# zhai-lw/L3AC

Hardware: AMD Instinct MI355X
Metric: audio samples/sec encode+decode, 1kbps@16kHz, batch 256; indices bit-exact (higher is better)
Workload: dtype f32

## Files before the change

include/l3ac_hip.h:

```cpp
#ifndef L3AC_HIP_H
#define L3AC_HIP_H

#include <stddef.h>
#include <stdint.h>

#ifdef __cplusplus
extern "C" {
#endif

#define L3AC_ABI_VERSION 5
#define L3AC_MAX_STAGES 8
#define L3AC_MAX_LEVELS 8

enum {
    L3AC_OK = 0,
    L3AC_EINVAL = -1,
    L3AC_EWEIGHT = -2,
    L3AC_EHIP = -3,
    L3AC_ENOMEM = -4,
    L3AC_ECOOP = -5,
};

typedef struct l3ac_config {
    int32_t abi_version;
// ... 94 lines not shown
int l3ac_op_enhance_up(l3ac_ctx* ctx, const char* enhance_block, const char* up_block, const float* x, int32_t batch,
                       int32_t frames, float* y, void* stream);
int l3ac_op_last_block(l3ac_ctx* ctx, const float* x, int32_t batch, int32_t frames, float* audio, void* stream);
int l3ac_op_legacy_unit(l3ac_ctx* ctx, int32_t unit, const float* x, int32_t batch, int32_t frames, float* y, void* stream);
int l3ac_op_head(l3ac_ctx* ctx, const float* x, int32_t batch, int32_t frames, float* audio, void* stream);
int l3ac_op_local_trans(l3ac_ctx* ctx, const char* block, const float* x, int32_t batch, int32_t frames, float* y,
                        void* stream);
int l3ac_op_encoder(l3ac_ctx* ctx, const float* audio, int32_t batch, int32_t samples, float* feature, void* stream);
int l3ac_op_en_encoder(l3ac_ctx* ctx, const float* feature, int32_t batch, int32_t frames, float* tokens, void* stream);
int l3ac_op_en_decoder(l3ac_ctx* ctx, const float* tokens, int32_t batch, int32_t n_tok, float* feature, void* stream);
int l3ac_op_decoder(l3ac_ctx* ctx, const float* feature, int32_t batch, int32_t frames, float* audio, void* stream);

int l3ac_op_snake(const float* x, float* y, int64_t rows, int32_t c, const float* alpha, int32_t mode, void* stream);
int l3ac_ctx_set_head_pretanh(l3ac_ctx* ctx, int32_t enable);

typedef struct l3ac_profile_entry {
    char name[64];
    int32_t launches;
    int32_t reserved;
    double ms_total;
    double flops;
    double bytes;
} l3ac_profile_entry;
int l3ac_profile_begin(void);
int l3ac_profile_end(l3ac_profile_entry* out, int32_t cap, int32_t* n_out);

int l3ac_gemm_f32(const float* a, int64_t lda, const float* w, const float* bias, float* c, int64_t ldc,
                  int64_t m, int32_t n, int32_t k, void* stream);

void l3ac_split3_host(const float* x, int64_t n, uint16_t* planes);
int l3ac_ctx_set_gemm_split(l3ac_ctx* ctx, int32_t enable);
int l3ac_ctx_set_option(l3ac_ctx* ctx, const char* name, int32_t value);
int l3ac_ctx_get_option(const l3ac_ctx* ctx, const char* name, int32_t* out);
int32_t l3ac_ctx_get_gemm_split(const l3ac_ctx* ctx);
int64_t l3ac_gemm_split_image_bytes(int32_t n, int32_t k);
int l3ac_gemm_split_image(const float* w, int32_t n, int32_t k, void* image, void* stream);
int l3ac_gemm_split_f32(const float* a, int64_t lda, const void* image, const float* bias, float* c, int64_t ldc,
                        int64_t m, int32_t n, int32_t k, void* stream);
int l3ac_gemm_split_f32_at(const float* a, int64_t lda, const void* image, const float* bias, float* c, int64_t ldc,
                           int64_t m, int32_t n, int32_t k, int32_t w256, void* stream);

#ifdef __cplusplus
}
#endif
#endif
```

l3ac_amd/_capi.py:

```python
from __future__ import annotations

import ctypes as C
from pathlib import Path

import os

LIB_PATH = Path(os.environ.get("L3AC_LIB_PATH") or Path(__file__).resolve().parent / "libl3ac_hip.so")
ABI_VERSION = 5
MAX_STAGES = 8
MAX_LEVELS = 8


class L3acError(RuntimeError):
    pass


class Config(C.Structure):
    _fields_ = [
        ("abi_version", C.c_int32),
        ("feature_dim", C.c_int32),
        ("n_enc", C.c_int32),
        ("enc_dims", C.c_int32 * MAX_STAGES),
        ("enc_depths", C.c_int32 * MAX_STAGES),
        ("compress_rates", C.c_int32 * MAX_STAGES),
# ... 31 lines not shown
    "l3ac_encode": (C.c_int, [_P, _P, _I32, _I32, _I64, _P, _P, _P, _P]),
    "l3ac_decode": (C.c_int, [_P, _P, _P, _I32, _I32, _P, _P]),
    "l3ac_encode_ragged": (C.c_int, [_P, _P, _I32, _I32, _I64, C.POINTER(_I32), _P, _P, _P, _P]),
    "l3ac_decode_ragged": (C.c_int, [_P, _P, _P, _I32, _I32, C.POINTER(_I32), _P, _P]),
    "l3ac_fsq_forward": (C.c_int, [_P, _I64, _I32, C.POINTER(_I32), _I32, _P, _P, _P, _P, _P, _P, _P, _P, _P]),
    "l3ac_fsq_quantize_act": (C.c_int, [_P, _I64, _I32, C.POINTER(_I32), _I32, _P, _P, _P, _P, _P, _P]),
    "l3ac_fsq_decode": (C.c_int, [_P, _I64, _I32, C.POINTER(_I32), _I32, _P, _P, _P, _P]),
    "l3ac_fsq_copy_ceiling": (C.c_int, [_P, _I64, _P, _P, _P, _P]),
    "l3ac_fsq_copy_ceiling_at": (C.c_int, [_P, _I64, _P, _P, _P, _I32, _P]),
    "l3ac_vq_argmin_scratch_bytes": (_I64, [_I64, _I32, _I32]),
    "l3ac_vq_argmin": (C.c_int, [_P, _I64, _P, _I32, _I32, _P, _P, _I64, _I32, _P]),
    "l3ac_op_first_block": (C.c_int, [_P, _P, _I32, _I32, _P, _P]),
    "l3ac_op_conv_unit": (C.c_int, [_P, C.c_char_p, _P, _I32, _I32, _P, _P]),
    "l3ac_op_down_layer": (C.c_int, [_P, C.c_char_p, _P, _I32, _I32, _P, _P]),
    "l3ac_op_conv_k3": (C.c_int, [_P, C.c_char_p, _P, _I32, _I32, _P, _P]),
    "l3ac_op_enhance": (C.c_int, [_P, C.c_char_p, _P, _I32, _I32, _P, _P]),
    "l3ac_op_up_layer": (C.c_int, [_P, C.c_char_p, _P, _I32, _I32, _P, _P]),
    "l3ac_op_enhance_up": (C.c_int, [_P, C.c_char_p, C.c_char_p, _P, _I32, _I32, _P, _P]),
    "l3ac_op_last_block": (C.c_int, [_P, _P, _I32, _I32, _P, _P]),
    "l3ac_op_legacy_unit": (C.c_int, [_P, _I32, _P, _I32, _I32, _P, _P]),
    "l3ac_op_head": (C.c_int, [_P, _P, _I32, _I32, _P, _P]),
    "l3ac_op_local_trans": (C.c_int, [_P, C.c_char_p, _P, _I32, _I32, _P, _P]),
    "l3ac_op_encoder": (C.c_int, [_P, _P, _I32, _I32, _P, _P]),
    "l3ac_op_en_encoder": (C.c_int, [_P, _P, _I32, _I32, _P, _P]),
    "l3ac_op_en_decoder": (C.c_int, [_P, _P, _I32, _I32, _P, _P]),
    "l3ac_op_decoder": (C.c_int, [_P, _P, _I32, _I32, _P, _P]),
    "l3ac_op_snake": (C.c_int, [_P, _P, _I64, _I32, _P, _I32, _P]),
    "l3ac_ctx_set_head_pretanh": (C.c_int, [_P, _I32]),
    "l3ac_gemm_f32": (C.c_int, [_P, _I64, _P, _P, _P, _I64, _I64, _I32, _I32, _P]),
    "l3ac_split3_host": (None, [_P, _I64, _P]),
    "l3ac_ctx_set_gemm_split": (C.c_int, [_P, _I32]),
    "l3ac_ctx_set_option": (C.c_int, [_P, C.c_char_p, _I32]),
    "l3ac_ctx_get_option": (C.c_int, [_P, C.c_char_p, C.POINTER(_I32)]),
    "l3ac_ctx_get_gemm_split": (_I32, [_P]),
    "l3ac_gemm_split_image_bytes": (_I64, [_I32, _I32]),
    "l3ac_gemm_split_image": (C.c_int, [_P, _I32, _I32, _P, _P]),
    "l3ac_gemm_split_f32": (C.c_int, [_P, _I64, _P, _P, _P, _I64, _I64, _I32, _I32, _P]),
    "l3ac_gemm_split_f32_at": (C.c_int, [_P, _I64, _P, _P, _P, _I64, _I64, _I32, _I32, _I32, _P]),
    "l3ac_pack_indices": (C.c_int, [_P, _I32, _I32, _I32, _P, _I32, _P]),
    "l3ac_unpack_indices": (C.c_int, [_P, _I32, _I32, _I32, _I32, _P, _P]),
    "l3ac_resample_length": (_I64, [_I32, _I32, _I64]),
    "l3ac_resample_bank": (_I64, [_I32, _I32, _P, _I64]),
    "l3ac_resample": (C.c_int, [_P, _I32, _I64, _I64, _I32, _I32, _P, _P, _I64, _P]),
    "l3ac_profile_begin": (C.c_int, []),
    "l3ac_profile_end": (C.c_int, [_P, _I32, C.POINTER(_I32)]),
}


class ProfileEntry(C.Structure):
    _fields_ = [("name", C.c_char * 64), ("launches", C.c_int32), ("reserved", C.c_int32),
                ("ms_total", C.c_double), ("flops", C.c_double), ("bytes", C.c_double)]


class profile:

    def __enter__(self):
        check(load_library().l3ac_profile_begin())
        self.entries = []
        return self

    def __exit__(self, *exc):
        buf = (ProfileEntry * 64)()
        n = C.c_int32(0)
        check(load_library().l3ac_profile_end(buf, 64, C.byref(n)))
        self.entries = [dict(name=buf[i].name.decode(), launches=buf[i].launches, ms_total=buf[i].ms_total,
                             flops=buf[i].flops, bytes=buf[i].bytes) for i in range(n.value)]
# ... 104 lines not shown
        return int(out.value)

    def coop_timeout_pending(self) -> int:
        out = _I64(0)
        check(self.lib.l3ac_coop_timeout_pending(self.handle, C.byref(out)))
        return int(out.value)

    def grn_min_norm(self, reset: bool = False) -> float:
        out = C.c_float(0.0)
        check(self.lib.l3ac_grn_min_norm(self.handle, int(reset), C.byref(out)))
        return float(out.value)

    @property
    def workspace_bytes(self) -> int:
        return self.lib.l3ac_workspace_bytes(self.handle)

    def reserve(self, batch: int, samples: int) -> None:
        check(self.lib.l3ac_reserve(self.handle, batch, samples))

    def set_gemm_split(self, enable: bool) -> None:
        check(self.lib.l3ac_ctx_set_gemm_split(self.handle, int(bool(enable))))

    def get_gemm_split(self) -> bool:
        return bool(self.lib.l3ac_ctx_get_gemm_split(self.handle))

    def set_option(self, name: str, value: int) -> None:
        check(self.lib.l3ac_ctx_set_option(self.handle, name.encode(), int(value)))

    def get_option(self, name: str) -> int:
        out = _I32(0)
        check(self.lib.l3ac_ctx_get_option(self.handle, name.encode(), C.byref(out)))
        return int(out.value)

    def set_head_pretanh(self, enable: bool) -> None:
        check(self.lib.l3ac_ctx_set_head_pretanh(self.handle, int(bool(enable))))
```

l3ac_amd/csrc/capi.hip:

```cpp
#include <algorithm>
#include <cmath>
#include <cstdarg>
#include <cstdlib>
#include <cstring>
#include <new>
#include <string>
#include <vector>

#include "network.hpp"
#include "kernels/split_bf16.hpp"

static thread_local std::string g_last_error;

void l3ac_set_error(const char* fmt, ...) {
    char buf[1024];
    va_list ap;
    va_start(ap, fmt);
    vsnprintf(buf, sizeof(buf), fmt, ap);
    va_end(ap);
    g_last_error = buf;
}

int l3ac_device_cu_count() {
    static std::atomic<int> cus[L3AC_MAX_DEVICES] = {};
// ... 97 lines not shown
template <class Map>
auto lookup(const Map& m, const char* name, const char* kind) -> decltype(m.begin()->second) {
    if (!name) {
        l3ac_set_error("null block name");
        return nullptr;
    }
    auto it = m.find(name);
    if (it == m.end()) {
        l3ac_set_error("no %s block named '%s'", kind, name);
        return nullptr;
    }
    return it->second;
}

struct Option {
    const char* name;
    int& (*field)(l3ac_ctx&);
    bool flag;
    int lo, hi, def;
    const char* env;
};
#define L3AC_FIELD(member) [](l3ac_ctx& c) -> int& { return c.member; }
const Option kOptions[] = {
    {"gemm_split", L3AC_FIELD(gemm_split), true, 0, 1, 1, "L3AC_GEMM_SPLIT"},
    {"head_pretanh", L3AC_FIELD(head_pretanh), true, 0, 1, 0, nullptr},
    {"narrow_ring", L3AC_FIELD(narrow_ring), false, 0, 2, 1, nullptr},
    {"wide_sliced", L3AC_FIELD(wide_sliced), false, 0, 2, 1, nullptr},
    {"unit_counter", L3AC_FIELD(unit_counter), false, 0, 3, 1, "L3AC_UNIT_COUNTER"},
    {"trans_coop", L3AC_FIELD(coop.enabled), true, 0, 1, 1, "L3AC_TRANS_COOP"},
    {"coop_timeout_ms", L3AC_FIELD(coop.timeout_ms), false, 1, 20000, 250, nullptr},
    {"down_fused", L3AC_FIELD(down_fused), false, 0, 2, 2, "L3AC_DOWN_FUSED"},
    {"gemm_w256", L3AC_FIELD(gemm_w256), false, 0, 2, 1, "L3AC_GEMM_W256"},
    {"unit_chunk_mb", L3AC_FIELD(unit_chunk_mb), false, 0, 65536, 192, "L3AC_UNIT_CHUNK_MB"},
};
#undef L3AC_FIELD

const Option* find_option(const char* name) {
    for (const Option& o : kOptions)
        if (std::strcmp(o.name, name) == 0) return &o;
    return nullptr;
}

int unknown_option(const char* who, const char* name) {
    std::string names;
    for (const Option& o : kOptions) names += std::string(names.empty() ? "" : ", ") + o.name;
    l3ac_set_error("%s: unknown option '%s' (%s; to set only: coop_release_claim, coop_test_fault)", who, name, names.c_str());
    return L3AC_EINVAL;
}

int initial_value(const Option& o) {
    const char* e = o.env ? std::getenv(o.env) : nullptr;
    return e ? std::atoi(e) : o.def;
}

int checked_value(const Option& o, int value) { return o.flag ? value != 0 : std::min(std::max(value, o.lo), o.hi); }

int set_checked(l3ac_ctx* ctx, const Option& o, int value, const char* who) {
    L3AC_REQUIRE(!(std::strcmp(o.name, "down_fused") == 0 && value == 1),
                 "%s: down_fused = 1 (the bf16x3 one-kernel down layers) was retired, DESIGN.md section 4; 2 (the default) is the one-kernel "
                 "form with the bits of 0, the GEMM + row kernel", who);
    o.field(*ctx) = checked_value(o, value);
    return L3AC_OK;
}

int ragged_plan(l3ac_ctx* ctx, hipStream_t s, RaggedPlan& p, int batch, int max_tok, const int32_t* n_tok, const int32_t* samples) {
    p.max_tok = max_tok;
// ... 576 lines not shown
    int rc = L3AC_OK;
    if (hipMemcpyAsync(inv, hi.data(), (size_t)c * sizeof(float), hipMemcpyHostToDevice, s) != hipSuccess) {
        l3ac_set_error("op_snake: upload failed");
        rc = L3AC_EHIP;
    }
    if (rc == L3AC_OK) rc = launch_snake(s, x, y, rows, c, alpha, inv, mode);
    (void)hipStreamSynchronize(s);
    (void)hipFree(inv);
    return rc;
}

int l3ac_ctx_set_option(l3ac_ctx* ctx, const char* name, int32_t value) {
    L3AC_REQUIRE(ctx != nullptr && name != nullptr, "set_option: null argument");
    if (std::strcmp(name, "coop_release_claim") == 0) {
        trans_coop_release(ctx->coop);
        return L3AC_OK;
    }
    if (std::strcmp(name, "coop_test_fault") == 0) {
        ctx->coop.fault_part = value - 1;
        return L3AC_OK;
    }
    const Option* o = find_option(name);
    return o ? set_checked(ctx, *o, value, "set_option") : unknown_option("set_option", name);
}

int l3ac_ctx_get_option(const l3ac_ctx* ctx, const char* name, int32_t* out) {
    L3AC_REQUIRE(ctx != nullptr && name != nullptr && out != nullptr, "get_option: null argument");
    const Option* o = find_option(name);
    if (!o) return unknown_option("get_option", name);
    *out = o->field(const_cast<l3ac_ctx&>(*ctx));
    return L3AC_OK;
}

int l3ac_ctx_set_gemm_split(l3ac_ctx* ctx, int32_t enable) { return l3ac_ctx_set_option(ctx, "gemm_split", enable); }
int32_t l3ac_ctx_get_gemm_split(const l3ac_ctx* ctx) { int32_t v = 0; return l3ac_ctx_get_option(ctx, "gemm_split", &v) == L3AC_OK ? v : 0; }

int64_t l3ac_gemm_split_image_bytes(int32_t n, int32_t k) {
    return (n > 0 && k > 0 && gemm_split_eligible(n, k)) ? gemm_split_image_bytes(n, k) : 0;
}

int l3ac_gemm_split_image(const float* w, int32_t n, int32_t k, void* image, void* stream) {
    L3AC_REQUIRE(gemm_split_eligible(n, k), "split image: shape n=%d k=%d is not eligible (n >= 192, k >= 32, k %% 8 == 0)", n, k);
    return launch_gemm_split_image((hipStream_t)stream, w, k, n, k, (unsigned char*)image);
}

int l3ac_gemm_split_f32_at(const float* a, int64_t lda, const void* image, const float* bias, float* c, int64_t ldc, int64_t m,
                           int32_t n, int32_t k, int32_t w256, void* stream) {
    L3AC_REQUIRE(w256 >= 0 && w256 <= 2, "split gemm: w256 = %d, not 0, 1 or 2", w256);
    GemmArgs g{};
    g.a = a; g.lda = lda; g.w_img = (const unsigned char*)image; g.c = c; g.ldc = ldc; g.m = m; g.n = n; g.k = k; g.bias = bias;
    g.epi = EPI_BIAS; g.w256 = w256;
    return launch_gemm_split((hipStream_t)stream, g);
}
int l3ac_gemm_split_f32(const float* a, int64_t lda, const void* image, const float* bias, float* c, int64_t ldc, int64_t m,
                        int32_t n, int32_t k, void* stream) {
    const Option& o = *find_option("gemm_w256");
    return l3ac_gemm_split_f32_at(a, lda, image, bias, c, ldc, m, n, k, checked_value(o, initial_value(o)), stream);
}

}
```

l3ac_amd/csrc/network.hip:

```cpp
#include "network.hpp"

#include <algorithm>
#include <cmath>
#include <cstring>

namespace {

constexpr int HEADS = 6;

struct Builder {
    std::unordered_map<std::string, const l3ac_tensor*> map;
    std::vector<float> host;
    float* dev = nullptr;
    size_t cap = 0;
    std::string err;
    struct GemmWeight { const float* d; int n, k; };
    std::vector<GemmWeight> gemm_ws;
    struct ExtraImage { std::vector<unsigned char> bytes; const unsigned char** target; };
    std::vector<ExtraImage> extra_imgs;
    const float* host_of(const float* d) const { return host.data() + (d - dev); }

    const float* gemm(const float* d, int n, int k) {
        if (d && gemm_split_eligible(n, k)) gemm_ws.push_back({d, n, k});
        return d;
    }
    const float* find(const std::string& name, int64_t numel) {
        auto it = map.find(name);
        if (it == map.end()) {
            if (err.empty()) err = "missing weight tensor '" + name + "'";
            return nullptr;
        }
        if (it->second->numel != numel) {
            if (err.empty())
// ... 696 lines not shown
    g.w = w.w; g.ldw = 3 * w.cin; g.c = y; g.ldc = w.cout; g.m = (int64_t)batch * frames; g.n = w.cout; g.k = 3 * w.cin;
    g.bias = w.b; g.epi = EPI_BIAS;
    (void)ctx;
    return gemm_on_route(ctx, s, g);
}

int run_enhance(l3ac_ctx* ctx, hipStream_t s, const EnhW& w, const float* x, float* y, int batch, int frames) {
    Workspace& ws = ctx->ws;
    const RaggedClips rc = ctx->rag ? ctx->rag->clips(frames) : RaggedClips{};
    L3AC_TRY(launch_enhance_branches(s, w.t, x, batch, frames, w.c, ws.yi, ctx->rag ? &rc : nullptr));
    L3AC_TRY(launch_enhance_stats(s, ws.yi, batch, frames, ws.stats, ctx->rag ? &rc : nullptr));
    RowArgs r{};
    r.x = x; r.y = y; r.batch = batch; r.frames_in = frames; r.frames_out = frames; r.c = w.c;
    r.src = SRC_GATE; r.norm = NORM_NONE; r.yi = ws.yi; r.stats = ws.stats; r.in_w = w.in_w; r.in_b = w.in_b;
    r.gate_w = w.gate_w; r.gate_b = w.gate_b;
    return launch_rows(s, r);
}

int run_up(l3ac_ctx* ctx, hipStream_t s, const UpW& w, const float* x, float* tmp, float* y, int batch, int frames) {
    GemmArgs g{};
    g.a = x; g.lda = w.cin; g.w = w.w; g.ldw = w.cin; g.c = tmp; g.ldc = w.cout; g.m = (int64_t)batch * frames; g.n = w.cout; g.k = w.cin;
    g.bias = w.b; g.epi = EPI_BIAS;
    L3AC_TRY(gemm_on_route(ctx, s, g));
    L3AC_TRY(rag_dup(ctx, s, tmp, batch, frames, w.cout));
    RowArgs r{};
    r.x = tmp; r.y = y; r.batch = batch; r.frames_in = frames; r.frames_out = (int64_t)frames * w.scale; r.c = w.cout;
    r.src = SRC_LERP; r.scale = w.scale; r.norm = NORM_CN; r.nw = w.nw; r.nb = w.nb; r.eps = 1e-8f;
    (void)ctx;
    return launch_rows(s, r);
}

static bool use_up_fused(const l3ac_ctx* ctx, const UpW& w) { return ctx->gemm_split && w.fused_img != nullptr; }

int run_enhance_up(l3ac_ctx* ctx, hipStream_t s, const EnhW& e, const UpW& w, float* x, float* tmp, float* y, int batch, int frames) {
    const bool wide_up = ctx->img(w.w) != nullptr && gemm_split_eligible(w.cout, w.cin);
    if (w.cin % 16 != 0 || e.c != w.cin || wide_up) {
        L3AC_REQUIRE(tmp != nullptr, "enhance_up: scratch missing");
        float* gated = x;
        if (x != y) {
            L3AC_REQUIRE((size_t)batch * frames * e.c <= ctx->ws.h_cap, "enhance_up: workspace too small for the gated rows");
            gated = ctx->ws.h;
        }
        L3AC_TRY(run_enhance(ctx, s, e, x, gated, batch, frames));
        return run_up(ctx, s, w, gated, tmp, y, batch, frames);
    }
    Workspace& ws = ctx->ws;
    const RaggedClips rc = ctx->rag ? ctx->rag->clips(frames) : RaggedClips{};
    L3AC_TRY(launch_enhance_branches(s, e.t, x, batch, frames, e.c, ws.yi, ctx->rag ? &rc : nullptr));
    L3AC_TRY(launch_enhance_stats(s, ws.yi, batch, frames, ws.stats, ctx->rag ? &rc : nullptr));
    if (use_up_fused(ctx, w) && x != y) {
        L3AC_TRY(rag_dup(ctx, s, x, batch, frames, e.c));
        L3AC_TRY(rag_dup(ctx, s, ws.yi, batch, frames, 4));
        return launch_up_fused(s, e, w, x, ws.yi, ws.stats, y, batch, frames);
    }
    L3AC_REQUIRE(tmp != nullptr, "enhance_up: scratch missing");
    GemmArgs g{};
    g.a = x; g.lda = w.cin; g.w = w.w; g.ldw = w.cin; g.c = tmp; g.ldc = w.cout; g.m = (int64_t)batch * frames; g.n = w.cout; g.k = w.cin;
    g.bias = w.b; g.epi = EPI_BIAS;
    g.gate_yi = ws.yi; g.gate_stats = ws.stats; g.gate_in_w = e.in_w; g.gate_in_b = e.in_b; g.gate_w = e.gate_w; g.gate_b = e.gate_b;
    g.gate_frames = frames;
    L3AC_TRY(launch_gemm(s, g));
    L3AC_TRY(rag_dup(ctx, s, tmp, batch, frames, w.cout));
    RowArgs r{};
    r.x = tmp; r.y = y; r.batch = batch; r.frames_in = frames; r.frames_out = (int64_t)frames * w.scale; r.c = w.cout;
    r.src = SRC_LERP; r.scale = w.scale; r.norm = NORM_CN; r.nw = w.nw; r.nb = w.nb; r.eps = 1e-8f;
    return launch_rows(s, r);
}

static bool last_block_fused(const l3ac_ctx* ctx) {
    int max_dil = 1;
    for (const LegacyW& l : ctx->legacy) max_dil = l.dil > max_dil ? l.dil : max_dil;
    return last_block_fused_supported(ctx->head.c, max_dil);
}

int run_legacy_unit(l3ac_ctx* ctx, hipStream_t s, const LegacyW& l, const float* x, float* y, int batch, int frames) {
    if (last_block_fused(ctx))
        return launch_legacy_unit_fused(s, l, x, y, batch, frames, ctx->gemm_split, ctx->unit_counter == 1 || ctx->unit_counter == 3 ? ctx->wide_counters + 4 : nullptr);
    Workspace& ws = ctx->ws;
    const int64_t rows = (int64_t)batch * frames;
    L3AC_TRY(launch_snake(s, x, ws.a, rows, l.c, l.a0, l.ia0));
    GemmArgs g{};
    g.a = ws.a; g.lda = l.c; g.taps = 7; g.dil = l.dil; g.cin = l.c; g.frames = frames;
    g.w = l.w1; g.ldw = 7 * l.c; g.c = ws.h; g.ldc = l.c; g.m = rows; g.n = l.c; g.k = 7 * l.c;
    g.bias = l.b1; g.epi = EPI_SNAKE; g.alpha = l.a1; g.inv_alpha = l.ia1;
    L3AC_TRY(gemm_on_route(ctx, s, g));
    GemmArgs g2{};
    g2.a = ws.h; g2.lda = l.c; g2.w = l.w2; g2.ldw = l.c; g2.c = y; g2.ldc = l.c; g2.m = rows; g2.n = l.c; g2.k = l.c;
    g2.bias = l.b2; g2.epi = EPI_BIAS_RES; g2.res = x; g2.ldres = l.c;
    return gemm_on_route(ctx, s, g2);
}

int run_head(l3ac_ctx* ctx, hipStream_t s, const float* x, float* audio, int batch, int frames) {
// ... 66 lines not shown
        RowArgs r{};
        r.x = x; r.y = ws.a; r.batch = batch; r.frames_in = frames; r.frames_out = frames; r.c = dim;
        r.src = SRC_PLAIN; r.norm = NORM_LN; r.nw = l.ln1w; r.nb = l.ln1b; r.eps = 1e-5f;
        L3AC_TRY(launch_rows(s, r));
        GemmArgs g{};
        g.a = ws.a; g.lda = dim; g.w = l.wqkv; g.ldw = dim; g.c = ws.h; g.ldc = 3 * ctx->inner; g.m = rows; g.n = 3 * ctx->inner; g.k = dim;
        g.epi = EPI_BIAS;
        L3AC_TRY(gemm_on_route(ctx, s, g));
        L3AC_TRY(launch_attention(s, ws.h, ws.a, w.bias_table, batch, frames, HEADS, ctx->dim_head, w.window));
        GemmArgs go{};
        go.a = ws.a; go.lda = ctx->inner; go.w = l.wout; go.ldw = ctx->inner; go.c = x; go.ldc = dim; go.m = rows; go.n = dim; go.k = ctx->inner;
        go.epi = EPI_BIAS_RES; go.res = x; go.ldres = dim;
        L3AC_TRY(gemm_on_route(ctx, s, go));
        r.nw = l.ln2w; r.nb = l.ln2b;
        L3AC_TRY(launch_rows(s, r));
        GemmArgs f1{};
        f1.a = ws.a; f1.lda = dim; f1.w = l.wff1; f1.ldw = dim; f1.c = ws.h; f1.ldc = ctx->ff_pad; f1.m = rows; f1.n = ctx->ff_n; f1.k = dim;
        f1.epi = EPI_GEGLU; f1.n_out = ctx->ff_inner;
        L3AC_TRY(gemm_on_route(ctx, s, f1));
        GemmArgs f2{};
        f2.a = ws.h; f2.lda = ctx->ff_pad; f2.w = l.wff2; f2.ldw = ctx->ff_pad; f2.c = x; f2.ldc = dim; f2.m = rows; f2.n = dim; f2.k = ctx->ff_pad;
        f2.epi = EPI_BIAS_RES; f2.res = x; f2.ldres = dim;
        L3AC_TRY(gemm_on_route(ctx, s, f2));
    }
    return L3AC_OK;
}

static inline void swap_bufs(float** a, float** b) {
    float* t = *a;
    *a = *b;
    *b = t;
}

int run_encoder(l3ac_ctx* ctx, hipStream_t s, const float* audio, int64_t audio_stride, int batch, int samples,
                int frames, float** cur, float** alt) {
    const l3ac_config& c = ctx->cfg;
    const RaggedClips rc = ctx->rag ? ctx->rag->clips(frames) : RaggedClips{};
    L3AC_TRY(launch_first_block(s, ctx->first, audio, audio_stride, batch, samples, frames, *cur, ctx->rag ? &rc : nullptr));
    int f = frames;
    for (int i = 0; i < c.n_enc; ++i) {
        L3AC_TRY(run_conv_units(ctx, s, ctx->enc_units[i], cur, alt, batch, f));
        if (i + 1 < c.n_enc) {
            L3AC_TRY(run_down(ctx, s, ctx->enc_down[i], *cur, *alt, batch, f));
            swap_bufs(cur, alt);
            f /= c.compress_rates[i];
        }
    }
    L3AC_TRY(rag_mask(ctx, s, *cur, batch, f, c.enc_dims[c.n_enc - 1], 1));
    L3AC_TRY(run_conv_k3(ctx, s, ctx->enc_out, *cur, *alt, batch, f));
    swap_bufs(cur, alt);
    return L3AC_OK;
}

int run_en_encoder(l3ac_ctx* ctx, hipStream_t s, int batch, int frames, float** cur, float** alt, int* n_tok) {
    if (ctx->en_enc.size() == 2) {
        L3AC_TRY(local_trans_step(ctx, s, ctx->en_enc[0], cur, alt, batch, frames));
        L3AC_TRY(run_down(ctx, s, ctx->en_down, *cur, *alt, batch, frames));
        swap_bufs(cur, alt);
        frames /= ctx->en_down.stride;
        L3AC_TRY(local_trans_step(ctx, s, ctx->en_enc[1], cur, alt, batch, frames));
    } else {
        L3AC_TRY(local_trans_step(ctx, s, ctx->en_enc[0], cur, alt, batch, frames));
    }
    *n_tok = frames;
    return L3AC_OK;
}

int run_en_decoder(l3ac_ctx* ctx, hipStream_t s, int batch, int n_tok, float** cur, float** alt, int* frames) {
    L3AC_TRY(local_trans_step(ctx, s, ctx->en_dec[0], cur, alt, batch, n_tok));
    int f = n_tok;
    if (ctx->en_dec.size() == 2) {
        const int r = ctx->cfg.en_coder_compress_rate;
        L3AC_TRY(rag_dup(ctx, s, *cur, batch, f, ctx->cfg.feature_dim));
        RowArgs u{};
        u.x = *cur; u.y = *alt; u.batch = batch; u.frames_in = f; u.frames_out = (int64_t)f * r; u.c = ctx->cfg.feature_dim;
        u.src = SRC_LERP; u.scale = r; u.norm = NORM_NONE;
        L3AC_TRY(launch_rows(s, u));
        swap_bufs(cur, alt);
        f *= r;
        L3AC_TRY(local_trans_step(ctx, s, ctx->en_dec[1], cur, alt, batch, f));
    }
    *frames = f;
    return L3AC_OK;
}

int run_decoder(l3ac_ctx* ctx, hipStream_t s, int batch, int frames, float** cur, float** alt, float* audio) {
    const l3ac_config& c = ctx->cfg;
    L3AC_TRY(rag_mask(ctx, s, *cur, batch, frames, ctx->dec_in.cin, 1));
    L3AC_TRY(run_conv_k3(ctx, s, ctx->dec_in, *cur, *alt, batch, frames));
    swap_bufs(cur, alt);
    int f = frames;
    for (int i = 0; i + 1 < c.n_dec; ++i) {
        L3AC_TRY(run_conv_units(ctx, s, ctx->dec_units[i], cur, alt, batch, f));
        if (use_up_fused(ctx, ctx->dec_up[i])) {
            L3AC_TRY(run_enhance_up(ctx, s, ctx->dec_enh[i], ctx->dec_up[i], *cur, nullptr, *alt, batch, f));
            swap_bufs(cur, alt);
        } else {
            L3AC_TRY(run_enhance_up(ctx, s, ctx->dec_enh[i], ctx->dec_up[i], *cur, *alt, *cur, batch, f));
        }
        f *= c.decode_rates[i];
    }
    return run_last_block(ctx, s, *cur, audio, batch, f);
}
```

l3ac_amd/csrc/network.hpp:

```cpp
#pragma once

#include <map>
#include <string>
#include <unordered_map>
#include <vector>

#include "kernels.hpp"

struct ConvUnitW {
    int c = 0;
    const float *dw_w, *dw_b, *ln_w, *ln_b, *w1, *b1, *alpha, *inv_alpha, *gamma, *beta, *w2, *b2;
    const unsigned char *w1_img = nullptr, *w2_img = nullptr;
    const unsigned char* wide_img = nullptr;
    const unsigned char* ring_img = nullptr;
};
struct DownW {
    int cin = 0, cout = 0, stride = 1;
    const float *w, *b, *nw = nullptr, *nb = nullptr;
    const unsigned char* exact_img = nullptr;
};
struct ConvK3W {
    int cin = 0, cout = 0;
    const float *w, *b;
};
// ... 44 lines not shown
    float *x0 = nullptr, *x1 = nullptr, *a = nullptr, *h = nullptr, *yi = nullptr, *stats = nullptr, *sumsq = nullptr;
    int* plan = nullptr;
    size_t x_cap = 0, a_cap = 0, h_cap = 0, yi_cap = 0, b_cap = 0;
    size_t bytes() const { return (2 * x_cap + a_cap + h_cap + yi_cap + 12 * b_cap) * sizeof(float); }
};

struct RaggedPlan {
    static constexpr int plan_ints() { return 3; }
    int max_tok = 0;
    std::vector<int> n_tok;
    std::vector<int> order;
    const int* n_dev = nullptr;
    const int* samples_dev = nullptr;
    const int* order_dev = nullptr;
    RaggedClips clips(int frames) const { return RaggedClips{n_dev, frames / max_tok, samples_dev}; }
};

struct l3ac_ctx {
    l3ac_config cfg{};
    int device = 0;
    int hop = 0, enc_rate = 1, dim_head = 0, inner = 0, ff_inner = 0, ff_pad = 0, ff_n = 0;
    float* arena = nullptr;
    size_t arena_floats = 0;
    unsigned char* img_arena = nullptr;
    size_t img_bytes = 0;
    std::unordered_map<const float*, const unsigned char*> split_img;
    int gemm_split, head_pretanh;
    int unit_counter;
    int wide_sliced;
    int narrow_ring;
    int down_fused;
    int gemm_w256;
    int unit_chunk_mb;
    const unsigned char* img(const float* w) const {
        if (!gemm_split) return nullptr;
        auto it = split_img.find(w);
        return it == split_img.end() ? nullptr : it->second;
    }

    FirstBlockW first{};
    std::vector<std::vector<ConvUnitW>> enc_units;
    std::vector<DownW> enc_down;
    ConvK3W enc_out{};
    std::vector<LocalTransW> en_enc;
    DownW en_down{};
    std::vector<LocalTransW> en_dec;
    const float *q_win = nullptr, *q_bin = nullptr, *q_wout = nullptr, *q_bout = nullptr;
    ConvK3W dec_in{};
    std::vector<std::vector<ConvUnitW>> dec_units;
    std::vector<EnhW> dec_enh;
    std::vector<UpW> dec_up;
    std::vector<LegacyW> legacy;
    HeadW head{};

    std::map<std::string, const ConvUnitW*> by_unit;
    std::map<std::string, const DownW*> by_down;
    std::map<std::string, const ConvK3W*> by_k3;
    std::map<std::string, const EnhW*> by_enh;
    std::map<std::string, const UpW*> by_up;
    std::map<std::string, const LocalTransW*> by_trans;

    Workspace ws;
    TransCoopState coop;
    int* bad_index_count = nullptr;
    int* wide_counters = nullptr;
    float* grn_min_sumsq = nullptr;
// ... 24 lines not shown
                          int frames, int sliced_mode, int* counters);
std::vector<unsigned char> conv_unit_wide_image(const float* w1, const float* w2, int c);
bool trans_stack_supported(int dim, int dim_head, int heads, int ff_inner, int frames, int window, int n_layers);
void trans_stack_layer_image(std::vector<unsigned char>& img, const float* wqkv, const float* wout, const float* wff1, int ff_n,
                             const float* wff2, int ff_pad);
int64_t trans_stack_layer_image_bytes();
int launch_trans_stack(hipStream_t s, const LocalTransW& w, float* x, int batch, int frames, float scale, TransCoopState* coop = nullptr);
size_t trans_stack_coop_bytes();
size_t trans_stack_coop_counter_offset();
size_t trans_stack_coop_counter_bytes();
int trans_stack_coop_max_batch();
bool trans_coop_admit(TransCoopState& st, int batch);
void trans_coop_release(TransCoopState& st);
int trans_coop_claimed_on_device(int device);
bool up_fused_supported(int cin, int cout);
std::vector<unsigned char> up_fused_image(const float* w, int cin, int cout);
int launch_up_fused(hipStream_t s, const EnhW& e, const UpW& w, const float* x, const float* yi, const float* stats, float* y, int batch, int frames);
bool down_exact_supported(int cin, int stride, int cout);
std::vector<unsigned char> down_exact_image(const float* w, int k, int cout);
int launch_down_exact(hipStream_t s, const DownW& w, const float* x, float* y, int batch, int frames_out);
bool last_block_fused_supported(int c, int max_dil);
std::vector<unsigned char> legacy_w1_image(const float* w1, int c);
std::vector<unsigned char> legacy_w2_image(const float* w2, int c);
int launch_legacy_unit_fused(hipStream_t s, const LegacyW& w, const float* x, float* y, int batch, int frames, bool split, int* counters);
int launch_head_fused(hipStream_t s, const HeadW& w, const float* x, int batch, int frames, float* audio, bool pretanh);
int conv_unit_step(l3ac_ctx* ctx, hipStream_t s, const ConvUnitW& w, float** cur, float** alt, int batch, int frames);
int run_conv_units(l3ac_ctx* ctx, hipStream_t s, const std::vector<ConvUnitW>& units, float** cur, float** alt, int batch, int frames);

int run_conv_unit(l3ac_ctx* ctx, hipStream_t s, const ConvUnitW& w, const float* x, float* y, int batch, int frames);
int run_down(l3ac_ctx* ctx, hipStream_t s, const DownW& w, const float* x, float* y, int batch, int frames);
int run_conv_k3(l3ac_ctx* ctx, hipStream_t s, const ConvK3W& w, const float* x, float* y, int batch, int frames);
int run_enhance(l3ac_ctx* ctx, hipStream_t s, const EnhW& w, const float* x, float* y, int batch, int frames);
int run_up(l3ac_ctx* ctx, hipStream_t s, const UpW& w, const float* x, float* tmp, float* y, int batch, int frames);
int run_enhance_up(l3ac_ctx* ctx, hipStream_t s, const EnhW& e, const UpW& w, float* x, float* tmp, float* y, int batch, int frames);
int run_last_block(l3ac_ctx* ctx, hipStream_t s, float* x, float* audio, int batch, int frames);
int run_legacy_unit(l3ac_ctx* ctx, hipStream_t s, const LegacyW& l, const float* x, float* y, int batch, int frames);
int run_head(l3ac_ctx* ctx, hipStream_t s, const float* x, float* audio, int batch, int frames);
int run_local_trans(l3ac_ctx* ctx, hipStream_t s, const LocalTransW& w, float* x, int batch, int frames);

int run_encoder(l3ac_ctx* ctx, hipStream_t s, const float* audio, int64_t audio_stride, int batch, int samples,
                int frames, float** cur, float** alt);
int run_en_encoder(l3ac_ctx* ctx, hipStream_t s, int batch, int frames, float** cur, float** alt, int* n_tok);
int run_en_decoder(l3ac_ctx* ctx, hipStream_t s, int batch, int n_tok, float** cur, float** alt, int* frames);
int run_decoder(l3ac_ctx* ctx, hipStream_t s, int batch, int frames, float** cur, float** alt, float* audio);
```

Before: 314.0 million.

## Run encoder head and decoder tail in clip groups sized to cache budget

Adds a stage-chaining path that splits the batch into clip groups and runs several consecutive high-resolution stages (first block, conv units, downsample in the encoder; enhance-up, legacy units and head in the decoder) group by group, so intermediates stay within a configurable budget that defaults to 144 MB. The goal is to keep activations resident in the large on-chip cache instead of streaming full-batch tensors through HBM between stages. The trade-off is more kernel launches with smaller grids, which can lower occupancy per launch. A negative option value switches to stage-major order, and a query API reports the group counts.

```diff
diff --git a/include/l3ac_hip.h b/include/l3ac_hip.h
--- a/include/l3ac_hip.h
+++ b/include/l3ac_hip.h
@@ -150,6 +150,7 @@
 int l3ac_ctx_set_gemm_split(l3ac_ctx* ctx, int32_t enable);
 int l3ac_ctx_set_option(l3ac_ctx* ctx, const char* name, int32_t value);
 int l3ac_ctx_get_option(const l3ac_ctx* ctx, const char* name, int32_t* out);
+int l3ac_stage_groups(const l3ac_ctx* ctx, int32_t batch, int32_t samples, int32_t* groups);
 int32_t l3ac_ctx_get_gemm_split(const l3ac_ctx* ctx);
 int64_t l3ac_gemm_split_image_bytes(int32_t n, int32_t k);
 int l3ac_gemm_split_image(const float* w, int32_t n, int32_t k, void* image, void* stream);
diff --git a/l3ac_amd/_capi.py b/l3ac_amd/_capi.py
--- a/l3ac_amd/_capi.py
+++ b/l3ac_amd/_capi.py
@@ -87,6 +87,7 @@
     "l3ac_ctx_set_gemm_split": (C.c_int, [_P, _I32]),
     "l3ac_ctx_set_option": (C.c_int, [_P, C.c_char_p, _I32]),
     "l3ac_ctx_get_option": (C.c_int, [_P, C.c_char_p, C.POINTER(_I32)]),
+    "l3ac_stage_groups": (C.c_int, [_P, _I32, _I32, C.POINTER(_I32)]),
     "l3ac_ctx_get_gemm_split": (_I32, [_P]),
     "l3ac_gemm_split_image_bytes": (_I64, [_I32, _I32]),
     "l3ac_gemm_split_image": (C.c_int, [_P, _I32, _I32, _P, _P]),
@@ -257,5 +258,10 @@
         check(self.lib.l3ac_ctx_get_option(self.handle, name.encode(), C.byref(out)))
         return int(out.value)
 
+    def stage_groups(self, batch: int, samples: int) -> tuple:
+        out = (_I32 * 2)()
+        check(self.lib.l3ac_stage_groups(self.handle, batch, samples, out))
+        return int(out[0]), int(out[1])
+
     def set_head_pretanh(self, enable: bool) -> None:
         check(self.lib.l3ac_ctx_set_head_pretanh(self.handle, int(bool(enable))))
diff --git a/l3ac_amd/csrc/capi.hip b/l3ac_amd/csrc/capi.hip
--- a/l3ac_amd/csrc/capi.hip
+++ b/l3ac_amd/csrc/capi.hip
@@ -153,6 +153,7 @@
     {"down_fused", L3AC_FIELD(down_fused), false, 0, 2, 2, "L3AC_DOWN_FUSED"},
     {"gemm_w256", L3AC_FIELD(gemm_w256), false, 0, 2, 1, "L3AC_GEMM_W256"},
     {"unit_chunk_mb", L3AC_FIELD(unit_chunk_mb), false, 0, 65536, 192, "L3AC_UNIT_CHUNK_MB"},
+    {"stage_chunk_mb", L3AC_FIELD(stage_chunk_mb), false, -65536, 65536, 144, "L3AC_STAGE_CHUNK_MB"},
 };
 #undef L3AC_FIELD
 
@@ -795,6 +796,16 @@
     return L3AC_OK;
 }
 
+int l3ac_stage_groups(const l3ac_ctx* ctx, int32_t batch, int32_t samples, int32_t* groups) {
+    L3AC_REQUIRE(ctx != nullptr && groups != nullptr && batch > 0 && samples > 0, "stage_groups: bad argument");
+    const int frames = (int)round_up64(samples, ctx->hop);
+    int enc = 1, dec = 1;
+    stage_group_counts(ctx, batch, samples, frames, frames / ctx->hop * ctx->cfg.en_coder_compress_rate, &enc, &dec);
+    groups[0] = enc;
+    groups[1] = dec;
+    return L3AC_OK;
+}
+
 int l3ac_ctx_set_gemm_split(l3ac_ctx* ctx, int32_t enable) { return l3ac_ctx_set_option(ctx, "gemm_split", enable); }
 int32_t l3ac_ctx_get_gemm_split(const l3ac_ctx* ctx) { int32_t v = 0; return l3ac_ctx_get_option(ctx, "gemm_split", &v) == L3AC_OK ? v : 0; }
 
diff --git a/l3ac_amd/csrc/network.hip b/l3ac_amd/csrc/network.hip
--- a/l3ac_amd/csrc/network.hip
+++ b/l3ac_amd/csrc/network.hip
@@ -1,4 +1,5 @@
 #include "network.hpp"
+#include "stage_groups.hpp"
 
 #include <algorithm>
 #include <cmath>
@@ -761,9 +762,16 @@
 
 static bool use_up_fused(const l3ac_ctx* ctx, const UpW& w) { return ctx->gemm_split && w.fused_img != nullptr; }
 
-int run_enhance_up(l3ac_ctx* ctx, hipStream_t s, const EnhW& e, const UpW& w, float* x, float* tmp, float* y, int batch, int frames) {
+static bool up_separate(const l3ac_ctx* ctx, const EnhW& e, const UpW& w) {
     const bool wide_up = ctx->img(w.w) != nullptr && gemm_split_eligible(w.cout, w.cin);
-    if (w.cin % 16 != 0 || e.c != w.cin || wide_up) {
+    return w.cin % 16 != 0 || e.c != w.cin || wide_up;
+}
+
+int run_enhance_up(l3ac_ctx* ctx, hipStream_t s, const EnhW& e, const UpW& w, float* x, float* tmp, float* y, int batch, int frames,
+                   int clip0) {
+    const bool separate = up_separate(ctx, e, w);
+    L3AC_REQUIRE(clip0 == 0 || (!separate && !ctx->rag && use_up_fused(ctx, w) && x != y), "enhance_up: a clip group needs the one-kernel form");
+    if (separate) {
         L3AC_REQUIRE(tmp != nullptr, "enhance_up: scratch missing");
         float* gated = x;
         if (x != y) {
@@ -775,18 +783,20 @@
     }
     Workspace& ws = ctx->ws;
     const RaggedClips rc = ctx->rag ? ctx->rag->clips(frames) : RaggedClips{};
-    L3AC_TRY(launch_enhance_branches(s, e.t, x, batch, frames, e.c, ws.yi, ctx->rag ? &rc : nullptr));
-    L3AC_TRY(launch_enhance_stats(s, ws.yi, batch, frames, ws.stats, ctx->rag ? &rc : nullptr));
+    float* yi = ws.yi + (int64_t)clip0 * frames * 4;
+    float* stats = ws.stats + (int64_t)clip0 * 8;
+    L3AC_TRY(launch_enhance_branches(s, e.t, x, batch, frames, e.c, yi, ctx->rag ? &rc : nullptr));
+    L3AC_TRY(launch_enhance_stats(s, yi, batch, frames, stats, ctx->rag ? &rc : nullptr));
     if (use_up_fused(ctx, w) && x != y) {
         L3AC_TRY(rag_dup(ctx, s, x, batch, frames, e.c));
-        L3AC_TRY(rag_dup(ctx, s, ws.yi, batch, frames, 4));
-        return launch_up_fused(s, e, w, x, ws.yi, ws.stats, y, batch, frames);
+        L3AC_TRY(rag_dup(ctx, s, yi, batch, frames, 4));
+        return launch_up_fused(s, e, w, x, yi, stats, y, batch, frames);
     }
     L3AC_REQUIRE(tmp != nullptr, "enhance_up: scratch missing");
     GemmArgs g{};
     g.a = x; g.lda = w.cin; g.w = w.w; g.ldw = w.cin; g.c = tmp; g.ldc = w.cout; g.m = (int64_t)batch * frames; g.n = w.cout; g.k = w.cin;
     g.bias = w.b; g.epi = EPI_BIAS;
-    g.gate_yi = ws.yi; g.gate_stats = ws.stats; g.gate_in_w = e.in_w; g.gate_in_b = e.in_b; g.gate_w = e.gate_w; g.gate_b = e.gate_b;
+    g.gate_yi = yi; g.gate_stats = stats; g.gate_in_w = e.in_w; g.gate_in_b = e.in_b; g.gate_w = e.gate_w; g.gate_b = e.gate_b;
     g.gate_frames = frames;
     L3AC_TRY(launch_gemm(s, g));
     L3AC_TRY(rag_dup(ctx, s, tmp, batch, frames, w.cout));
@@ -919,13 +929,174 @@
     *b = t;
 }
 
+namespace {
+
+struct ChainStep {
+    enum Kind { FIRST, UNIT, DOWN, UP, LEGACY, HEAD } kind;
+    const ConvUnitW* unit;
+    int idx;
+    int frames;
+};
+
+struct Chain {
+    std::vector<ChainStep> steps;
+    int64_t heaviest = 0;
+    int64_t clip_floats = 0;
+    int next_stage = 0, frames_out = 0;
+    void add(ChainStep::Kind kind, const ConvUnitW* unit, int idx, int frames, int64_t bytes, int64_t out_floats) {
+        steps.push_back(ChainStep{kind, unit, idx, frames});
+        heaviest = std::max(heaviest, bytes);
+        clip_floats = std::max(clip_floats, out_floats);
+    }
+};
+
+struct ChainIO {
+    const float* in;
+    int64_t in_stride;
+    float* out;
+    int64_t out_stride;
+    float *p, *q;
+    int samples;
+};
+
+bool units_out_of_place(const l3ac_ctx* ctx, const std::vector<ConvUnitW>& units) {
+    for (const ConvUnitW& u : units)
+        if (ctx->cfg.grn_exact || use_wide(ctx, u) || !conv_unit_fused_supported(u.c)) return false;
+    return true;
+}
+
+StageGroups chain_groups(const l3ac_ctx* ctx, const Chain& ch, int batch) {
+    const int mb = ctx->stage_chunk_mb;
+    if (ch.steps.empty() || ctx->rag) return stage_groups(batch, 0, 0);
+    return stage_groups(batch, ch.heaviest, mb < 0 ? -mb : mb);
+}
+
+Chain decoder_tail_chain(const l3ac_ctx* ctx, int batch, int frames, int* first_stage) {
+    const l3ac_config& c = ctx->cfg;
+    Chain ch;
+    *first_stage = -1;
+    const int last = c.n_dec - 2;
+    if (ctx->stage_chunk_mb == 0 || ctx->rag || last < 0 || !last_block_fused(ctx)) return ch;
+    auto up_ok = [&](int j) { return use_up_fused(ctx, ctx->dec_up[j]) && !up_separate(ctx, ctx->dec_enh[j], ctx->dec_up[j]); };
+    int i0 = last + 1;
+    for (int j = last; j >= 0 && up_ok(j); --j) {
+        i0 = j;
+        if (!units_out_of_place(ctx, ctx->dec_units[j])) break;
+    }
+    if (i0 > last) return ch;
+    std::vector<int64_t> f(c.n_dec, frames);
+    for (int j = 1; j < c.n_dec; ++j) f[j] = f[j - 1] * c.decode_rates[j - 1];
+    auto up_bytes = [&](int j) { return stage_bytes_resample(f[j], ctx->dec_up[j].cin, f[j + 1], ctx->dec_up[j].cout); };
+    const int64_t budget = (int64_t)std::abs(ctx->stage_chunk_mb) << 20;
+    while (i0 < last && batch * up_bytes(i0) <= budget) ++i0;
+    for (int j = i0; j <= last; ++j) {
+        if (j > i0)
+            for (const ConvUnitW& u : ctx->dec_units[j]) ch.add(ChainStep::UNIT, &u, j, (int)f[j], stage_bytes_unit(f[j], u.c), f[j] * u.c);
+        ch.add(ChainStep::UP, nullptr, j, (int)f[j], up_bytes(j), f[j + 1] * ctx->dec_up[j].cout);
+    }
+    const int64_t fl = f[c.n_dec - 1];
+    for (size_t k = 0; k < ctx->legacy.size(); ++k)
+        ch.add(ChainStep::LEGACY, nullptr, (int)k, (int)fl, stage_bytes_legacy(fl, ctx->legacy[k].c), fl * ctx->legacy[k].c);
+    ch.add(ChainStep::HEAD, nullptr, 0, (int)fl, stage_bytes_resample(fl, ctx->head.c, fl, 1), 0);
+    *first_stage = i0;
+    return ch;
+}
+
+Chain encoder_head_chain(const l3ac_ctx* ctx, int batch, int samples, int frames) {
+    const l3ac_config& c = ctx->cfg;
+    Chain ch;
+    if (ctx->stage_chunk_mb == 0 || ctx->rag) return ch;
+    auto down_bytes = [&](int i, int64_t f) {
+        const DownW& d = ctx->enc_down[i];
+        return stage_bytes_resample(f, d.cin, f / d.stride, d.cout);
+    };
+    int n = 0;
+    int64_t f = frames;
+    std::vector<int64_t> fr;
+    while (n + 1 < c.n_enc && units_out_of_place(ctx, ctx->enc_units[n]) && use_down_exact(ctx, ctx->enc_down[n]) &&
+           f % ctx->enc_down[n].stride == 0) {
+        fr.push_back(f);
+        f /= c.compress_rates[n];
+        ++n;
+    }
+    const int64_t budget = (int64_t)std::abs(ctx->stage_chunk_mb) << 20;
+    while (n > 0 && batch * down_bytes(n - 1, fr[n - 1]) <= budget) --n;
+    if (n == 0) return ch;
+    ch.add(ChainStep::FIRST, nullptr, 0, frames, stage_bytes_resample(samples, 1, frames, ctx->first.d0), (int64_t)frames * ctx->first.d0);
+    for (int i = 0; i < n; ++i) {
+        for (const ConvUnitW& u : ctx->enc_units[i]) ch.add(ChainStep::UNIT, &u, i, (int)fr[i], stage_bytes_unit(fr[i], u.c), fr[i] * u.c);
+        ch.add(ChainStep::DOWN, nullptr, i, (int)fr[i], down_bytes(i, fr[i]), i + 1 < n ? fr[i] / ctx->enc_down[i].stride * ctx->enc_down[i].cout : 0);
+    }
+    ch.next_stage = n;
+    ch.frames_out = (int)(fr[n - 1] / c.compress_rates[n - 1]);
+    return ch;
+}
+
+int chain_step(l3ac_ctx* ctx, hipStream_t s, const ChainStep& st, const ChainIO& io, const float* x, float* y, int b0, int nb) {
+    switch (st.kind) {
+        case ChainStep::FIRST: return launch_first_block(s, ctx->first, x, io.in_stride, nb, io.samples, st.frames, y, nullptr);
+        case ChainStep::UNIT: {
+            float *cur = const_cast<float*>(x), *alt = y;
+            L3AC_TRY(conv_unit_step(ctx, s, *st.unit, &cur, &alt, nb, st.frames));
+            L3AC_REQUIRE(cur == y, "stage chain: a unit ran in place");
+            return L3AC_OK;
+        }
+        case ChainStep::DOWN: return run_down(ctx, s, ctx->enc_down[st.idx], x, y, nb, st.frames);
+        case ChainStep::UP:
+            return run_enhance_up(ctx, s, ctx->dec_enh[st.idx], ctx->dec_up[st.idx], const_cast<float*>(x), nullptr, y, nb, st.frames, b0);
+        case ChainStep::LEGACY: return run_legacy_unit(ctx, s, ctx->legacy[st.idx], x, y, nb, st.frames);
+        case ChainStep::HEAD: return run_head(ctx, s, x, y, nb, st.frames);
+    }
+    return L3AC_EINVAL;
+}
+
+int run_chain(l3ac_ctx* ctx, hipStream_t s, const Chain& ch, const StageGroups& sg, const ChainIO& io) {
+    const bool stage_major = ctx->stage_chunk_mb < 0;
+    const int n = (int)ch.steps.size();
+    const size_t need = (size_t)(stage_major ? sg.batch : sg.max_count()) * ch.clip_floats;
+    L3AC_REQUIRE(need <= ctx->ws.x_cap && need <= ctx->ws.a_cap, "stage chain: workspace too small for a clip group");
+    auto step = [&](int k, int g) -> int {
+        const int b0 = sg.first(g), nb = sg.count(g);
+        const int64_t off = stage_major ? (int64_t)b0 * ch.clip_floats : 0;
+        const float* x = k == 0 ? io.in + b0 * io.in_stride : ((k & 1) ? io.p : io.q) + off;
+        float* y = k + 1 == n ? io.out + b0 * io.out_stride : ((k & 1) ? io.q : io.p) + off;
+        return chain_step(ctx, s, ch.steps[k], io, x, y, b0, nb);
+    };
+    if (stage_major) {
+        for (int k = 0; k < n; ++k)
+            for (int g = 0; g < sg.groups; ++g) L3AC_TRY(step(k, g));
+    } else {
+        for (int g = 0; g < sg.groups; ++g)
+            for (int k = 0; k < n; ++k) L3AC_TRY(step(k, g));
+    }
+    return L3AC_OK;
+}
+
+}
+
+void stage_group_counts(const l3ac_ctx* ctx, int batch, int samples, int enc_frames, int dec_frames, int* enc, int* dec) {
+    int first_stage = -1;
+    *enc = chain_groups(ctx, encoder_head_chain(ctx, batch, samples, enc_frames), batch).groups;
+    *dec = chain_groups(ctx, decoder_tail_chain(ctx, batch, dec_frames, &first_stage), batch).groups;
+}
+
 int run_encoder(l3ac_ctx* ctx, hipStream_t s, const float* audio, int64_t audio_stride, int batch, int samples,
                 int frames, float** cur, float** alt) {
     const l3ac_config& c = ctx->cfg;
     const RaggedClips rc = ctx->rag ? ctx->rag->clips(frames) : RaggedClips{};
-    L3AC_TRY(launch_first_block(s, ctx->first, audio, audio_stride, batch, samples, frames, *cur, ctx->rag ? &rc : nullptr));
-    int f = frames;
-    for (int i = 0; i < c.n_enc; ++i) {
+    int f = frames, i = 0;
+    const Chain head = encoder_head_chain(ctx, batch, samples, frames);
+    const StageGroups sg = chain_groups(ctx, head, batch);
+    if (sg.groups > 1) {
+        const DownW& d = ctx->enc_down[head.next_stage - 1];
+        const ChainIO io{audio, audio_stride, *cur, (int64_t)head.frames_out * d.cout, *alt, ctx->ws.a, samples};
+        L3AC_TRY(run_chain(ctx, s, head, sg, io));
+        i = head.next_stage;
+        f = head.frames_out;
+    } else {
+        L3AC_TRY(launch_first_block(s, ctx->first, audio, audio_stride, batch, samples, frames, *cur, ctx->rag ? &rc : nullptr));
+    }
+    for (; i < c.n_enc; ++i) {
         L3AC_TRY(run_conv_units(ctx, s, ctx->enc_units[i], cur, alt, batch, f));
         if (i + 1 < c.n_enc) {
             L3AC_TRY(run_down(ctx, s, ctx->enc_down[i], *cur, *alt, batch, f));
@@ -976,9 +1147,15 @@
     L3AC_TRY(rag_mask(ctx, s, *cur, batch, frames, ctx->dec_in.cin, 1));
     L3AC_TRY(run_conv_k3(ctx, s, ctx->dec_in, *cur, *alt, batch, frames));
     swap_bufs(cur, alt);
-    int f = frames;
+    int f = frames, first_stage = -1;
+    const Chain tail = decoder_tail_chain(ctx, batch, frames, &first_stage);
+    const StageGroups sg = chain_groups(ctx, tail, batch);
     for (int i = 0; i + 1 < c.n_dec; ++i) {
         L3AC_TRY(run_conv_units(ctx, s, ctx->dec_units[i], cur, alt, batch, f));
+        if (sg.groups > 1 && i == first_stage) {
+            const ChainIO io{*cur, (int64_t)f * ctx->dec_up[i].cin, audio, tail.steps.back().frames, *alt, ctx->ws.a, 0};
+            return run_chain(ctx, s, tail, sg, io);
+        }
         if (use_up_fused(ctx, ctx->dec_up[i])) {
             L3AC_TRY(run_enhance_up(ctx, s, ctx->dec_enh[i], ctx->dec_up[i], *cur, nullptr, *alt, batch, f));
             swap_bufs(cur, alt);
diff --git a/l3ac_amd/csrc/network.hpp b/l3ac_amd/csrc/network.hpp
--- a/l3ac_amd/csrc/network.hpp
+++ b/l3ac_amd/csrc/network.hpp
@@ -100,6 +100,7 @@
     int down_fused;
     int gemm_w256;
     int unit_chunk_mb;
+    int stage_chunk_mb;
     const unsigned char* img(const float* w) const {
         if (!gemm_split) return nullptr;
         auto it = split_img.find(w);
@@ -190,7 +191,8 @@
 int run_conv_k3(l3ac_ctx* ctx, hipStream_t s, const ConvK3W& w, const float* x, float* y, int batch, int frames);
 int run_enhance(l3ac_ctx* ctx, hipStream_t s, const EnhW& w, const float* x, float* y, int batch, int frames);
 int run_up(l3ac_ctx* ctx, hipStream_t s, const UpW& w, const float* x, float* tmp, float* y, int batch, int frames);
-int run_enhance_up(l3ac_ctx* ctx, hipStream_t s, const EnhW& e, const UpW& w, float* x, float* tmp, float* y, int batch, int frames);
+int run_enhance_up(l3ac_ctx* ctx, hipStream_t s, const EnhW& e, const UpW& w, float* x, float* tmp, float* y, int batch, int frames,
+                   int clip0 = 0);
 int run_last_block(l3ac_ctx* ctx, hipStream_t s, float* x, float* audio, int batch, int frames);
 int run_legacy_unit(l3ac_ctx* ctx, hipStream_t s, const LegacyW& l, const float* x, float* y, int batch, int frames);
 int run_head(l3ac_ctx* ctx, hipStream_t s, const float* x, float* audio, int batch, int frames);
@@ -201,3 +203,4 @@
 int run_en_encoder(l3ac_ctx* ctx, hipStream_t s, int batch, int frames, float** cur, float** alt, int* n_tok);
 int run_en_decoder(l3ac_ctx* ctx, hipStream_t s, int batch, int n_tok, float** cur, float** alt, int* frames);
 int run_decoder(l3ac_ctx* ctx, hipStream_t s, int batch, int frames, float** cur, float** alt, float* audio);
+void stage_group_counts(const l3ac_ctx* ctx, int batch, int samples, int enc_frames, int dec_frames, int* enc, int* dec);
diff --git a/l3ac_amd/csrc/stage_groups.hpp b/l3ac_amd/csrc/stage_groups.hpp
--- /dev/null
+++ b/l3ac_amd/csrc/stage_groups.hpp
@@ -0,0 +1,31 @@
+#pragma once
+
+#include <cstdint>
+
+inline int64_t stage_bytes_unit(int64_t frames, int c) { return frames * c * 4 * 2; }
+inline int64_t stage_bytes_legacy(int64_t frames, int c) { return frames * c * 4 * 3; }
+inline int64_t stage_bytes_resample(int64_t frames_in, int c_in, int64_t frames_out, int c_out) {
+    return (frames_in * c_in + frames_out * c_out) * 4;
+}
+
+inline int stage_group_clips(int batch, int64_t bytes_per_clip, int chunk_mb) {
+    if (batch < 1) return 1;
+    if (chunk_mb <= 0 || bytes_per_clip <= 0) return batch;
+    const int64_t g = ((int64_t)chunk_mb << 20) / bytes_per_clip;
+    return g < 1 ? 1 : g > batch ? batch : (int)g;
+}
+
+struct StageGroups {
+    int batch = 0, groups = 1;
+    int first(int k) const { return (int)((int64_t)k * (batch / groups)) + (k < batch % groups ? k : batch % groups); }
+    int count(int k) const { return batch / groups + (k < batch % groups ? 1 : 0); }
+    int max_count() const { return (batch + groups - 1) / groups; }
+};
+
+inline StageGroups stage_groups(int batch, int64_t bytes_per_clip, int chunk_mb) {
+    StageGroups g;
+    g.batch = batch < 1 ? 1 : batch;
+    const int clips = stage_group_clips(g.batch, bytes_per_clip, chunk_mb);
+    g.groups = (g.batch + clips - 1) / clips;
+    return g;
+}
```

New measurement: 294.7 million (median of 2 runs). 6.1% lower.
